# VITA-Group/MLSP

Measured on AMD Instinct MI355X. Metric: points/sec fwd+bwd, DGCNN+MLSP B=32 N=1024 k=20, higher is better.
Workload: dtype f32; 1 GPU; DGCNN encoder + 3 MLSP heads + losses, fwd+bwd+Adam, B=32/GPU N=1024 k=20 fp32 (BASELINE.json configs[1]), dropout 0.5, BN train; global_batch=32, points_per_cloud=1024, k=20, parallelism=dp1

## Files before the change

mlsp_amd/csrc/api.hip:

```cpp
#include "common.h"
#include "../../include/mlsp_hip.h"

#define CHECK(x) do { int _r = (x); if (_r != MLSP_OK) return _r; } while (0)
#define SLAB_BOUND_FLOATS ((size_t)16 << 20)

#include <mutex>
#include <unordered_map>
hipError_t mlsp_lds_limit(const void* fn, size_t lds) {
    static std::mutex mu;
    static std::unordered_map<uint64_t, size_t> raised;
    int dev = 0;
    (void)hipGetDevice(&dev);
    const uint64_t key = (uint64_t)(uintptr_t)fn * 64u + (uint64_t)(dev & 63);
    std::lock_guard<std::mutex> lk(mu);
    auto it = raised.find(key);
    if (it != raised.end() && it->second >= lds) return hipSuccess;
    const hipError_t e = hipFuncSetAttribute(fn, hipFuncAttributeMaxDynamicSharedMemorySize, (int)lds);
    if (e == hipSuccess) raised[key] = lds;
    return e;
}

extern "C" {

int mlsp_abi_version(void) { return MLSP_ABI_VERSION; }
// ... 157 lines not shown
    PREC_SCOPE(precision);
    if (!x || !idx || !W || !gamma || !beta || !out || !uv || !msel || !argsel || !s1 || !bn_save) return MLSP_ERR_ARG;
    if (B <= 0 || N <= 0 || C <= 0 || Cout <= 0 || k <= 0 || k > 255 || ldx < C || ldo < Cout) return MLSP_ERR_ARG;
    const int P = B * N;
    Workspace w(ws, ws_bytes);
    float* Wd = Wd_out ? Wd_out : w.take<float>((size_t)2 * Cout * C);
    int nparts = edge_reduce_parts(P);
    double* part = w.take<double>((size_t)nparts * 2 * Cout);
    GemmOpts so; take_slab(w, so, gemm_slab_floats(P, 2 * Cout, C));
    if (!w.ok()) return MLSP_ERR_WORKSPACE;
    float* scale = bn_save, *shift = bn_save + Cout, *mean = bn_save + 2 * Cout, *invstd = bn_save + 3 * Cout;
    if (!training) {
        if (!run_mean || !run_var) return MLSP_ERR_ARG;
        CHECK(launch_build_wd_eval(st, W, Cout, C, Wd, Cout, gamma, beta, run_mean, run_var, bn_save, 0, nullptr, nullptr, nullptr, nullptr, nullptr, eps));
    } else CHECK(launch_build_wd(st, W, Cout, C, Wd, (C >= 128 && C % 32 == 0 && build_wd_leaves_bound(Cout, C)) ? amax_reserve(Wd, 2 * Cout, C, C) : nullptr));
    CHECK(launch_gemm(st, false, true, P, 2 * Cout, C, x, ldx, Wd, C, uv, 2 * Cout, so));
    {
        const int tok = prof_cls_begin(st, MLSP_PROF_EDGE_REDUCE);
        const int rc = launch_edge_reduce(st, uv, idx, gamma, P, N, Cout, k, msel, argsel, s1, part, &nparts);
        prof_cls_end(st, tok, (double)P * (Cout * 4.0 + k * 4.0 + Cout * 9.0));
        if (rc != MLSP_OK) return rc;
    }
    if (training) {
        CHECK(launch_bn_finalize(st, part, nparts, (double)P * k, Cout, gamma, beta, run_mean, run_var, momentum, eps, scale,
                                 shift, mean, invstd, amax_offered_output(out, P, Cout, ldo, Cout)));
    }
    CHECK(launch_edge_select_act(st, msel, uv, P, Cout, scale, shift, act, slope, out, ldo));
    return MLSP_OK;
}

int mlsp_edgeconv_bwd_f32(const float* dOut, int lddo, const float* x, int ldx, const int32_t* rev_off, const int32_t* rev_ent,
                          const float* W, const float* out, int ldo, const float* uv, const float* msel, const uint8_t* argsel,
                          const float* s1, const float* bn_save, const float* Wd_in, int act, float slope, int training, int B, int N, int C,
                          int Cout, int k, float* dx, int lddx, int dx_accumulate, float* dW, float* dgamma, float* dbeta, int precision, void* ws,
                          size_t ws_bytes, mlsp_stream_t st) {
    PREC_SCOPE(precision);
    if (!dOut || !x || !rev_off || !rev_ent || !W || !out || !uv || !msel || !argsel || !s1 || !bn_save || !dW || !dgamma ||
        !dbeta)
        return MLSP_ERR_ARG;
    if (B <= 0 || N <= 0 || C <= 0 || Cout <= 0 || k <= 0 || ldx < C || lddo < Cout || ldo < Cout || (dx && lddx < C)) return MLSP_ERR_ARG;
    const int P = B * N;
    Workspace w(ws, ws_bytes);
    float* Wd = Wd_in ? nullptr : w.take<float>((size_t)2 * Cout * C);
    float* dWd = w.take<float>((size_t)2 * Cout * C);
    float* gz = w.take<float>((size_t)P * Cout);
    float* duv = w.take<float>((size_t)P * 2 * Cout);
    int nparts = bn_parts_max(P);
    double* part = w.take<double>((size_t)nparts * 2 * Cout);
    float* mean_dz = w.take<float>(Cout);
    float* mean_dzy = w.take<float>(Cout);
    GemmOpts so; take_slab(w, so, gemm_slab_floats(P, C, 2 * Cout), gemm_slab_floats(2 * Cout, C, P));
    if (!w.ok()) return MLSP_ERR_WORKSPACE;
    const float* scale = bn_save, *mean = bn_save + 2 * Cout, *invstd = bn_save + 3 * Cout;
    float* duv_amax = (C % 128 == 0 && edge_bwd_leaves_duv_bound(dOut, out, msel, uv, s1, argsel, Cout, scale, mean, invstd, gz, duv, lddo, ldo))
                          ? amax_reserve(duv, P, 2 * Cout, 2 * Cout) : nullptr;
    CHECK(launch_edge_bwd_reduce(st, dOut, out, msel, uv, P, Cout, mean, invstd, act, slope, part, lddo, ldo, duv_amax));
    CHECK(launch_bn_bwd_finalize(st, part, edge_bwd_reduce_parts(P, Cout, dOut, out, msel, uv, mean, invstd, lddo, ldo), (double)P * k, Cout,
                                 dgamma, dbeta, mean_dz, mean_dzy));
    const float* mdz = training ? mean_dz : nullptr;
    CHECK(launch_edge_bwd_point(st, dOut, out, uv, s1, P, Cout, k, scale, mean, invstd, mdz, mean_dzy, act, slope, gz, duv, lddo, ldo, duv_amax));
    CHECK(launch_edge_bwd_gather(st, gz, argsel, uv, rev_off, rev_ent, P, N, Cout, scale, mean, invstd, mdz, mean_dzy, duv, duv_amax));
    const float* Wdc = Wd_in;
    if (!Wdc && dx) { CHECK(launch_build_wd(st, W, Cout, C, Wd)); Wdc = Wd; }
    GemmOpts od = so; od.accumulate = dx_accumulate != 0;
    if (dx) CHECK(launch_gemm(st, false, false, P, C, 2 * Cout, duv, 2 * Cout, Wdc, C, dx, lddx, od));
    bool unfolded = false;
    GemmOpts ow = so; ow.unfold_dw = dW; ow.unfolded = &unfolded;
    CHECK(launch_gemm(st, true, false, 2 * Cout, C, P, duv, 2 * Cout, x, ldx, dWd, C, ow));
    if (!unfolded) CHECK(launch_unbuild_wd(st, dWd, Cout, C, dW));
    return MLSP_OK;
}

int mlsp_tnet_edge_fwd_f32(const float* x, int ldx, const int32_t* idx, const float* W1, const float* gamma1, const float* beta1,
                           float* run_mean1, float* run_var1, const float* W2, const float* gamma2, const float* beta2,
                           float* run_mean2, float* run_var2, float momentum, float eps, float slope, int training, int B, int N,
                           int C, int C1, int C2, int k, float* out, float* uv, float* s1, float* bn1_save, float* zsel,
                           uint8_t* argsel, float* bn2_save, int precision, void* ws, size_t ws_bytes, mlsp_stream_t st) {
    PREC_SCOPE(precision);
    if (!x || !idx || !W1 || !gamma1 || !beta1 || !W2 || !gamma2 || !beta2 || !out || !uv || !s1 || !bn1_save || !zsel || !argsel ||
        !bn2_save)
        return MLSP_ERR_ARG;
    if (B <= 0 || N <= 0 || C <= 0 || k <= 0 || ldx < C) return MLSP_ERR_ARG;
    if (C1 != 64 || C2 != 128 || tnet_points_per_tile(k) <= 0) return MLSP_ERR_UNSUPPORTED;
    const int P = B * N;
    Workspace w(ws, ws_bytes);
    float* Wd = w.take<float>((size_t)2 * C1 * C);
    float* msel = w.take<float>((size_t)P * C1);
    uint8_t* arg1 = w.take<uint8_t>((size_t)P * C1);
    int np1 = edge_reduce_parts(P), np2 = tnet_fwd_parts(B, N, k);
    double* part = w.take<double>((size_t)(np1 > np2 ? np1 : np2) * 2 * C2);
    GemmOpts so; take_slab(w, so, gemm_slab_floats(P, 2 * C1, C));
    if (!w.ok()) return MLSP_ERR_WORKSPACE;
    if (!training) {
        if (!run_mean1 || !run_var1 || !run_mean2 || !run_var2) return MLSP_ERR_ARG;
        CHECK(launch_build_wd_eval(st, W1, C1, C, Wd, C1, gamma1, beta1, run_mean1, run_var1, bn1_save, C2, gamma2, beta2, run_mean2, run_var2, bn2_save, eps));
    } else CHECK(launch_build_wd(st, W1, C1, C, Wd));
    CHECK(launch_gemm(st, false, true, P, 2 * C1, C, x, ldx, Wd, C, uv, 2 * C1, so));
    CHECK(launch_edge_reduce(st, uv, idx, gamma1, P, N, C1, k, msel, arg1, s1, part, &np1));
    if (training) {
        CHECK(launch_bn_finalize(st, part, np1, (double)P * k, C1, gamma1, beta1, run_mean1, run_var1, momentum, eps, bn1_save,
                                 bn1_save + C1, bn1_save + 2 * C1, bn1_save + 3 * C1));
    }
    {
        const int tok = prof_cls_begin(st, MLSP_PROF_TNET_FWD);
        const int rc = launch_tnet_edge_fwd(st, uv, idx, bn1_save, W2, gamma2, P, N, k, slope, zsel, argsel, part);
        prof_cls_end(st, tok, 2.0 * P * (double)k * C1 * C2);
        if (rc != MLSP_OK) return rc;
    }
    if (training) {
        CHECK(launch_bn_finalize(st, part, np2, (double)P * k, C2, gamma2, beta2, run_mean2, run_var2, momentum, eps, bn2_save,
                                 bn2_save + C2, bn2_save + 2 * C2, bn2_save + 3 * C2, amax_offered_output(out, P, C2, C2, C2)));
    }
    CHECK(launch_tnet_out(st, zsel, bn2_save, P, slope, out));
    return MLSP_OK;
// ... 782 lines not shown
```

mlsp_amd/csrc/edge.hip:

```cpp
#include "common.h"
#include <math.h>
#include <cstdlib>

#define EDGE_PTS_PER_WAVE 16

__global__ __launch_bounds__(256) void build_wd_kernel(const float* __restrict__ W, int Cout, int C, float* __restrict__ Wd, float* __restrict__ amax) {
    __shared__ float sm[4];
    int t = blockIdx.x * blockDim.x + threadIdx.x;
    float m = 0.f;
    if (t < Cout * C) {
        int o = t / C, c = t % C;
        float wa = W[(size_t)o * 2 * C + c], wb = W[(size_t)o * 2 * C + C + c];
        Wd[(size_t)o * C + c] = wa;
        Wd[(size_t)(Cout + o) * C + c] = wb - wa;
        m = fmaxf(fabsf(wa), fabsf(wb - wa));
    }
    if (!amax) return;
#pragma unroll
    for (int o = 1; o < 64; o <<= 1) m = fmaxf(m, __shfl_xor(m, o, 64));
    if ((threadIdx.x & 63) == 0) sm[threadIdx.x >> 6] = m;
    __syncthreads();
    if (threadIdx.x == 0) amax[blockIdx.x] = fmaxf(fmaxf(sm[0], sm[1]), fmaxf(sm[2], sm[3]));
    if (blockIdx.x == 0 && threadIdx.x >= gridDim.x) amax[threadIdx.x] = 0.f;
}
// ... 281 lines not shown
        for (int s0 = 0; s0 < KMAX; s0 += KC) {
            int jr[KC];
            if (EXACT && (KC % 4) == 0) {
#pragma unroll
                for (int s4 = 0; s4 < KC / 4; ++s4) {
                    const int4 t = *(const int4*)(irow + s0 + 4 * s4);
                    jr[4 * s4] = t.x; jr[4 * s4 + 1] = t.y; jr[4 * s4 + 2] = t.z; jr[4 * s4 + 3] = t.w;
                }
            } else {
#pragma unroll
                for (int s = 0; s < KC; ++s) jr[s] = (EXACT || s0 + s < k) ? irow[s0 + s] : 0;
            }
#pragma unroll
            for (int s = 0; s < KC; ++s) {
                if (EXACT || s0 + s < k) {
                    const f32x4 t = *(const f32x4*)(Us + jr[s] * CS + 4 * q);
                    const f32x2 ta = {t[0], t[1]}, tb = {t[2], t[3]};
                    s1a += ta; s1b += tb;
                    s2a = __builtin_elementwise_fma(ta, ta, s2a); s2b = __builtin_elementwise_fma(tb, tb, s2b);
#pragma unroll
                    for (int e = 0; e < 4; ++e) {
                        const bool take = (s0 + s == 0) || (t[e] > best[e]);
                        best[e] = take ? t[e] : best[e]; bs[e] = take ? s0 + s : bs[e];
                    }
                }
            }
        }
        const float s1[4] = {s1a[0] * sg[0], s1a[1] * sg[1], s1b[0] * sg[2], s1b[1] * sg[3]}, s2[4] = {s2a[0], s2a[1], s2b[0], s2b[1]};
        f32x4 b4, s4;
        uint32_t a4 = 0;
#pragma unroll
        for (int e = 0; e < 4; ++e) {
            b4[e] = best[e] * sg[e]; s4[e] = s1[e]; a4 |= (uint32_t)(bs[e] & 255) << (8 * e);
            ps[e] += (double)s1[e] + (double)k * v[e];
            pq[e] += (double)s2[e] + 2.0 * (double)v[e] * s1[e] + (double)k * v[e] * v[e];
        }
        *(f32x4*)(msel + i * Cout + c0 + 4 * q) = b4;
        *(f32x4*)(s1out + i * Cout + c0 + 4 * q) = s4;
        *(uint32_t*)(argsel + i * Cout + c0 + 4 * q) = a4;
    }
    __syncthreads();
    double* red = (double*)esm;
#pragma unroll
    for (int e = 0; e < 4; ++e) { red[(0 * PL + pl) * CS + 4 * q + e] = ps[e]; red[(1 * PL + pl) * CS + 4 * q + e] = pq[e]; }
    __syncthreads();
    if (tid < 2 * CS) {
        const int which = tid / CS, c = tid % CS;
        double a = 0.0;
        for (int u = 0; u < PL; ++u) a += red[(which * PL + u) * CS + c];
        part[((size_t)(b * psplit + ch) * 2 + which) * Cout + c0 + c] = a;
    }
}

__device__ __forceinline__ void edge_amax_raise(float* __restrict__ amax, float m) {
    __shared__ float wm[4];
#pragma unroll
    for (int o = 1; o < 64; o <<= 1) m = fmaxf(m, __shfl_xor(m, o, 64));
    if ((threadIdx.x & 63) == 0) wm[threadIdx.x >> 6] = m;
    __syncthreads();
    if (threadIdx.x == 0) atomicMax((unsigned int*)amax + (blockIdx.x & 255), __float_as_uint(fmaxf(fmaxf(wm[0], wm[1]), fmaxf(wm[2], wm[3]))));
}

template <int LR>
__global__ __launch_bounds__(256) void edge_bwd_gather_vec_kernel(const float* __restrict__ gz, const uint8_t* __restrict__ argsel,
                                                                  const float* __restrict__ uv, const int* __restrict__ rev_off,
                                                                  const int* __restrict__ rev_ent, int P, int N,
                                                                  const float* __restrict__ scale, const float* __restrict__ mean,
                                                                  const float* __restrict__ invstd,
                                                                  const float* __restrict__ mean_dz,
                                                                  const float* __restrict__ mean_dzy, float* __restrict__ duv,
                                                                  float* __restrict__ duv_amax) {
    constexpr int Cout = LR * 4, NP = 64 / LR;
    const int lane = threadIdx.x & 63;
    const int w = __builtin_amdgcn_readfirstlane(threadIdx.x >> 6);
    int j = blockIdx.x * 4 + w;
    if (N % 4 == 0) {
        int cloud, chunk;
        xcd_cloud_map(blockIdx.x, N / 4, P / N, cloud, chunk);
        j = cloud * N + chunk * 4 + w;
    }
    float pm = 0.f;
    if (j < P) {
        const int sub = lane / LR, c = (lane % LR) * 4;
        const int base = (j / N) * N;
        const int e0 = rev_off[j], e1 = rev_off[j + 1];
        const int ld = 2 * Cout;
        float A[4] = {0, 0, 0, 0}, Bc[4] = {0, 0, 0, 0};
        if (mean_dz) {
#pragma unroll
            for (int e = 0; e < 4; ++e) { float sc = scale[c + e]; A[e] = sc * mean_dz[c + e]; Bc[e] = sc * invstd[c + e] * mean_dzy[c + e]; }
        }
        float acc[4] = {0, 0, 0, 0};
        for (int ec = e0; ec < e1; ec += 64) {
            const int nent = min(64, e1 - ec);
            const int entv = lane < nent ? rev_ent[ec + lane] : 0;
            for (int t0 = 0; t0 < nent; t0 += NP) {
                const int t = t0 + sub;
                const bool ok = t < nent;
                const int ent = __shfl(entv, ok ? t : 0, 64);
                const int i = base + (ent >> 8), slot = ent & 255;
                const f32x4 g = *(const f32x4*)(gz + (size_t)i * Cout + c);
                const uint32_t a4 = *(const uint32_t*)(argsel + (size_t)i * Cout + c);
                const f32x4 v = *(const f32x4*)(uv + (size_t)i * ld + Cout + c);
#pragma unroll
                for (int e = 0; e < 4; ++e) {
                    float ge = (((a4 >> (8 * e)) & 255) == (uint32_t)slot) ? g[e] : 0.f;
                    acc[e] += ok ? (ge - Bc[e] * v[e]) : 0.f;
                }
            }
        }
#pragma unroll
        for (int o = LR; o < 64; o <<= 1)
#pragma unroll
// ... 117 lines not shown
    }
}

__global__ __launch_bounds__(256) void edge_select_act_vec_kernel(const float* __restrict__ msel, const float* __restrict__ uv,
                                                                  size_t total4, int C4, const float* __restrict__ scale,
                                                                  const float* __restrict__ shift, int act, float slope,
                                                                  float* __restrict__ out, int ldo) {
    for (size_t v = blockIdx.x * (size_t)blockDim.x + threadIdx.x; v < total4; v += (size_t)gridDim.x * blockDim.x) {
        const size_t i = v / C4; const int c = (int)(v % C4) * 4;
        const f32x4 m = *(const f32x4*)(msel + v * 4), vv = *(const f32x4*)(uv + i * 8 * C4 + 4 * C4 + c);
        const f32x4 sc = *(const f32x4*)(scale + c), sh = *(const f32x4*)(shift + c);
        f32x4 o;
#pragma unroll
        for (int e = 0; e < 4; ++e) o[e] = lrelu_or_relu(fmaf(m[e] + vv[e], sc[e], sh[e]), act, slope);
        *(f32x4*)(out + i * ldo + c) = o;
    }
}

__global__ __launch_bounds__(256) void edge_bwd_point_vec_kernel(const float* __restrict__ dOut, const float* __restrict__ out,
                                                                 const float* __restrict__ uv, const float* __restrict__ s1,
                                                                 size_t total4, int C4, int k, const float* __restrict__ scale,
                                                                 const float* __restrict__ mean, const float* __restrict__ invstd,
                                                                 const float* __restrict__ mean_dz, const float* __restrict__ mean_dzy,
                                                                 int act, float slope, float* __restrict__ gz,
                                                                 float* __restrict__ duv, int lddo, int ldo,
                                                                 float* __restrict__ duv_amax) {
    const float fk = (float)k;
    float pm = 0.f;
    for (size_t v = blockIdx.x * (size_t)blockDim.x + threadIdx.x; v < total4; v += (size_t)gridDim.x * blockDim.x) {
        const size_t i = v / C4; const int c = (int)(v % C4) * 4;
        const f32x4 d4 = *(const f32x4*)(dOut + i * lddo + c), o4 = *(const f32x4*)(out + i * ldo + c);
        const f32x4 sc = *(const f32x4*)(scale + c);
        f32x4 g, dv;
#pragma unroll
        for (int e = 0; e < 4; ++e) {
            float d = d4[e];
            if (act && !(o4[e] > 0.f)) d *= (act == 1 ? 0.f : slope);
            g[e] = sc[e] * d; dv[e] = g[e];
        }
        if (mean_dz) {
            const f32x4 vv = *(const f32x4*)(uv + i * 8 * C4 + 4 * C4 + c), s4 = *(const f32x4*)(s1 + v * 4);
#pragma unroll
            for (int e = 0; e < 4; ++e) {
                float A = sc[e] * mean_dz[c + e], Bc = sc[e] * invstd[c + e] * mean_dzy[c + e];
                dv[e] = g[e] - fk * A - Bc * (s4[e] + fk * (vv[e] - mean[c + e]));
            }
        }
        *(f32x4*)(gz + v * 4) = g;
        *(f32x4*)(duv + i * 8 * C4 + 4 * C4 + c) = dv;
#pragma unroll
        for (int e = 0; e < 4; ++e) pm = fmaxf(pm, fabsf(dv[e]));
    }
    if (duv_amax) edge_amax_raise(duv_amax, pm);
}

__global__ __launch_bounds__(256) void edge_bwd_gather_kernel(const float* __restrict__ gz, const uint8_t* __restrict__ argsel,
                                                              const float* __restrict__ uv, const int* __restrict__ rev_off,
                                                              const int* __restrict__ rev_ent, int P, int N, int Cout,
                                                              const float* __restrict__ scale, const float* __restrict__ mean,
                                                              const float* __restrict__ invstd,
                                                              const float* __restrict__ mean_dz,
                                                              const float* __restrict__ mean_dzy, float* __restrict__ duv) {
    const int lane = threadIdx.x & 63;
    const int w = __builtin_amdgcn_readfirstlane(threadIdx.x >> 6);
    const int j = blockIdx.x * 4 + w;
    if (j >= P) return;
    const int base = (j / N) * N;
    const int e0 = rev_off[j], e1 = rev_off[j + 1];
    const int ld = 2 * Cout;
    for (int c = lane; c < Cout; c += 64) {
        float A = 0.f, Bc = 0.f;
        if (mean_dz) { float sc = scale[c]; A = sc * mean_dz[c]; Bc = sc * invstd[c] * mean_dzy[c]; }
        float acc = 0.f;
        for (int e = e0; e < e1; ++e) {
            int ent = rev_ent[e];
            int i = base + (ent >> 8), slot = ent & 255;
            size_t t = (size_t)i * Cout + c;
            float g = (argsel[t] == slot) ? gz[t] : 0.f;
            acc += g - Bc * uv[(size_t)i * ld + Cout + c];
        }
        float u = uv[(size_t)j * ld + c];
        duv[(size_t)j * ld + c] = acc - (float)(e1 - e0) * (A + Bc * (u - mean[c]));
    }
}

__global__ __launch_bounds__(256) void graph_feature_fwd_kernel(const float* __restrict__ x, const int* __restrict__ idx,
                                                                int P, int N, int C, int k, float* __restrict__ F) {
    size_t total = (size_t)P * k * C;
    for (size_t t = blockIdx.x * (size_t)blockDim.x + threadIdx.x; t < total; t += (size_t)gridDim.x * blockDim.x) {
        int c = (int)(t % C);
        size_t e = t / C;
        size_t i = e / k;
        int j = (int)(i / N) * N + idx[e];
        float xi = x[i * C + c];
        F[e * 2 * C + c] = x[(size_t)j * C + c] - xi;
        F[e * 2 * C + C + c] = xi;
    }
}

__global__ __launch_bounds__(256) void graph_feature_bwd_kernel(const float* __restrict__ dF, const int* __restrict__ rev_off,
                                                                const int* __restrict__ rev_ent, int P, int N, int C, int k,
                                                                float* __restrict__ dx) {
    size_t total = (size_t)P * C;
    for (size_t t = blockIdx.x * (size_t)blockDim.x + threadIdx.x; t < total; t += (size_t)gridDim.x * blockDim.x) {
        int c = (int)(t % C);
        size_t i = t / C;
// ... 72 lines not shown
        int psplit = 1;
        while (psplit < 8 && (B * nsl * psplit < 512 || (N / psplit) * k * 2 > 16 * 1024) && N % (psplit * 2) == 0) psplit *= 2;
        const size_t lds = (size_t)N * ELDS_CS * sizeof(float) + align_up((size_t)((N + psplit - 1) / psplit) * k * 2, 16);
        if (lds <= 150 * 1024 && B * psplit <= edge_reduce_parts(P) && lds >= (size_t)2 * (256 / (ELDS_CS / 4)) * ELDS_CS * sizeof(double)) {
            auto kern = k == 20 ? edge_reduce_lds_kernel<20, true> : k <= 20 ? edge_reduce_lds_kernel<20, false> : k <= 32 ? edge_reduce_lds_kernel<32, false>
                      : k == 40 ? edge_reduce_lds_kernel<40, true> : edge_reduce_lds_kernel<40, false>;
            if (lds > 64 * 1024) {
                hipError_t e = mlsp_lds_limit((const void*)kern, lds);
                if (e != hipSuccess) return (int)e;
            }
            hipLaunchKernelGGL(kern, dim3(B * nsl * psplit), dim3(256), lds, st, uv, idx, gamma, B, N, k, Cout, psplit, msel, argsel, s1, part);
            if (nparts_used) *nparts_used = B * psplit;
            return mlsp_launch_status();
        }
    }
    if (al && (Cout == 64 || Cout == 128 || Cout == 256)) {
        dim3 g(edge_reduce_parts(P)), b(256);
        if (Cout == 64) hipLaunchKernelGGL((edge_reduce_vec_kernel<16>), g, b, 0, st, uv, idx, gamma, P, N, k, msel, argsel, s1, part);
        else if (Cout == 128) hipLaunchKernelGGL((edge_reduce_vec_kernel<32>), g, b, 0, st, uv, idx, gamma, P, N, k, msel, argsel, s1, part);
        else hipLaunchKernelGGL((edge_reduce_vec_kernel<64>), g, b, 0, st, uv, idx, gamma, P, N, k, msel, argsel, s1, part);
        return mlsp_launch_status();
    }
    size_t lds = (size_t)8 * Cout * sizeof(double);
    if (lds > 64 * 1024) return MLSP_ERR_UNSUPPORTED;
    hipLaunchKernelGGL(edge_reduce_kernel, dim3(edge_reduce_parts(P)), dim3(256), lds, st, uv, idx, gamma, P, N, Cout, k,
                       msel, argsel, s1, part);
    return mlsp_launch_status();
}
int launch_edge_select_act(hipStream_t st, const float* msel, const float* uv, int P, int Cout, const float* scale,
                           const float* shift, int act, float slope, float* out, int ldo) {
    if (Cout % 4 == 0 && ldo % 4 == 0 && ((((uintptr_t)msel | (uintptr_t)uv | (uintptr_t)out | (uintptr_t)scale | (uintptr_t)shift) & 15) == 0)) {
        size_t t4 = (size_t)P * Cout / 4;
        hipLaunchKernelGGL(edge_select_act_vec_kernel, dim3(ew_blocks2(t4)), dim3(256), 0, st, msel, uv, t4, Cout / 4, scale, shift,
                           act, slope, out, ldo);
        return mlsp_launch_status();
    }
    hipLaunchKernelGGL(edge_select_act_kernel, dim3(ew_blocks2((size_t)P * Cout)), dim3(256), 0, st, msel, uv, P, Cout, scale,
                       shift, act, slope, out, ldo);
    return mlsp_launch_status();
}
static bool edge_bwd_reduce_vec_ok(const float* dOut, const float* out, const float* msel, const float* uv, int Cout, const float* mean,
                                   const float* invstd, int lddo, int ldo) {
    return Cout % 4 == 0 && Cout <= 1024 && 256 % (Cout / 4) == 0 && lddo % 4 == 0 && ldo % 4 == 0 &&
           ((((uintptr_t)dOut | (uintptr_t)out | (uintptr_t)msel | (uintptr_t)uv | (uintptr_t)mean | (uintptr_t)invstd) & 15) == 0);
}
static bool edge_bwd_point_vec_ok(const float* dOut, const float* out, const float* uv, const float* s1, int Cout, const float* scale,
                                  const float* gz, const float* duv, int lddo, int ldo) {
    return Cout % 4 == 0 && lddo % 4 == 0 && ldo % 4 == 0 &&
           ((((uintptr_t)dOut | (uintptr_t)out | (uintptr_t)uv | (uintptr_t)s1 | (uintptr_t)gz | (uintptr_t)duv | (uintptr_t)scale) & 15) == 0);
}
static bool edge_bwd_gather_vec_ok(const float* gz, const uint8_t* argsel, const float* uv, int Cout, const float* duv) {
    return (((uintptr_t)uv | (uintptr_t)gz | (uintptr_t)duv) & 15) == 0 && (((uintptr_t)argsel) & 3) == 0 && (Cout == 64 || Cout == 128 || Cout == 256);
}
bool edge_bwd_leaves_duv_bound(const float* dOut, const float* out, const float* msel, const float* uv, const float* s1, const uint8_t* argsel,
                               int Cout, const float* scale, const float* mean, const float* invstd, const float* gz, const float* duv,
                               int lddo, int ldo) {
    return edge_bwd_reduce_vec_ok(dOut, out, msel, uv, Cout, mean, invstd, lddo, ldo) &&
           edge_bwd_point_vec_ok(dOut, out, uv, s1, Cout, scale, gz, duv, lddo, ldo) && edge_bwd_gather_vec_ok(gz, argsel, uv, Cout, duv);
}
int launch_edge_bwd_reduce(hipStream_t st, const float* dOut, const float* out, const float* msel, const float* uv, int P,
                           int Cout, const float* mean, const float* invstd, int act, float slope, double* part, int lddo, int ldo,
                           float* duv_amax) {
    if (edge_bwd_reduce_vec_ok(dOut, out, msel, uv, Cout, mean, invstd, lddo, ldo)) {
        hipLaunchKernelGGL(edge_bwd_reduce_vec_kernel, dim3((P + EVROWS - 1) / EVROWS), dim3(256), 0, st, dOut, out, msel, uv, P, Cout,
                           mean, invstd, act, slope, part, lddo, ldo, duv_amax);
        return mlsp_launch_status();
    }
    hipLaunchKernelGGL(edge_bwd_reduce_kernel, dim3((Cout + 63) / 64, (P + 511) / 512), dim3(256), 0, st, dOut, out, msel, uv,
                       P, Cout, mean, invstd, act, slope, part, lddo, ldo);
    return mlsp_launch_status();
}
int launch_edge_bwd_point(hipStream_t st, const float* dOut, const float* out, const float* uv, const float* s1, int P,
                          int Cout, int k, const float* scale, const float* mean, const float* invstd, const float* mean_dz,
                          const float* mean_dzy, int act, float slope, float* gz, float* duv, int lddo, int ldo, float* duv_amax) {
    if (edge_bwd_point_vec_ok(dOut, out, uv, s1, Cout, scale, gz, duv, lddo, ldo)) {
        size_t t4 = (size_t)P * Cout / 4;
        hipLaunchKernelGGL(edge_bwd_point_vec_kernel, dim3(ew_blocks2(t4)), dim3(256), 0, st, dOut, out, uv, s1, t4, Cout / 4, k, scale,
                           mean, invstd, mean_dz, mean_dzy, act, slope, gz, duv, lddo, ldo, duv_amax);
        return mlsp_launch_status();
    }
    hipLaunchKernelGGL(edge_bwd_point_kernel, dim3(ew_blocks2((size_t)P * Cout)), dim3(256), 0, st, dOut, out, uv, s1, P, Cout,
                       k, scale, mean, invstd, mean_dz, mean_dzy, act, slope, gz, duv, lddo, ldo);
    return mlsp_launch_status();
}
int launch_edge_bwd_gather(hipStream_t st, const float* gz, const uint8_t* argsel, const float* uv, const int* rev_off,
                           const int* rev_ent, int P, int N, int Cout, const float* scale, const float* mean,
                           const float* invstd, const float* mean_dz, const float* mean_dzy, float* duv, float* duv_amax) {
    if (edge_bwd_gather_vec_ok(gz, argsel, uv, Cout, duv)) {
        dim3 g((P + 3) / 4), b(256);
        if (Cout == 64) hipLaunchKernelGGL((edge_bwd_gather_vec_kernel<16>), g, b, 0, st, gz, argsel, uv, rev_off, rev_ent, P, N, scale, mean, invstd, mean_dz, mean_dzy, duv, duv_amax);
        else if (Cout == 128) hipLaunchKernelGGL((edge_bwd_gather_vec_kernel<32>), g, b, 0, st, gz, argsel, uv, rev_off, rev_ent, P, N, scale, mean, invstd, mean_dz, mean_dzy, duv, duv_amax);
        else hipLaunchKernelGGL((edge_bwd_gather_vec_kernel<64>), g, b, 0, st, gz, argsel, uv, rev_off, rev_ent, P, N, scale, mean, invstd, mean_dz, mean_dzy, duv, duv_amax);
        return mlsp_launch_status();
    }
    hipLaunchKernelGGL(edge_bwd_gather_kernel, dim3((P + 3) / 4), dim3(256), 0, st, gz, argsel, uv, rev_off, rev_ent, P, N,
                       Cout, scale, mean, invstd, mean_dz, mean_dzy, duv);
    return mlsp_launch_status();
}
int launch_graph_feature_fwd(hipStream_t st, const float* x, const int* idx, int P, int N, int C, int k, float* F) {
    hipLaunchKernelGGL(graph_feature_fwd_kernel, dim3(ew_blocks2((size_t)P * k * C)), dim3(256), 0, st, x, idx, P, N, C, k, F);
    return mlsp_launch_status();
}
int launch_graph_feature_bwd(hipStream_t st, const float* dF, const int* rev_off, const int* rev_ent, int P, int N, int C,
                             int k, float* dx) {
    hipLaunchKernelGGL(graph_feature_bwd_kernel, dim3(ew_blocks2((size_t)P * C)), dim3(256), 0, st, dF, rev_off, rev_ent, P, N,
                       C, k, dx);
    return mlsp_launch_status();
}
```

mlsp_amd/csrc/launchers.h:

```cpp
#pragma once

hipError_t mlsp_lds_limit(const void* fn, size_t lds);

int gemm_precision_mode();
float* amax_reserve(const float* X, long rows, int cols, int ld);
float* amax_offered_output(const float* out, long rows, int cols, int ld, int need);
int launch_slab_reduce(hipStream_t st, const float* slab, float* C, int M, int N, int ldc, int nsplit, float* unfold_dw = nullptr,
                       bool* unfolded = nullptr);
int gemm_stat_parts(int M, int N, int K);
int gemm_panel_rows(int M, int N, int K);
size_t gemm_slab_floats(int M, int N, int K);
int prof_cls_begin(hipStream_t st, int cls);
void prof_cls_end(hipStream_t st, int token, double work);
bool gemm_xf_supported(bool ta, bool tb, int M, int N, int K, const float* A, int lda, const float* B, int ldb, int which);
int gemm_bs_parts(int M, int N, int K, int lda, int ldb, int ldc);
bool gemm_dy_supported(bool ta, bool tb, int M, int N, int K, const float* A, int lda, const float* B, int ldb);
bool gemm_xf_on_split(bool ta, bool tb, int M, int N, int K, int which);
int launch_gemm(hipStream_t st, bool ta, bool tb, int M, int N, int K, const float* A, int lda, const float* B, int ldb, float* C, int ldc,
                const GemmOpts& o = GemmOpts());
int launch_gemm_mx(hipStream_t st, bool ta, bool tb, int M, int N, int K, const void* A, int a_bf16, int lda, const void* B, int b_bf16, int ldb,
                   void* C, int c_bf16, int ldc, const GemmOpts& o = GemmOpts());

int launch_knn(hipStream_t st, const float* x, int ld, int B, int N, int C, int k, int* idx, float* xx_ws, void* planes, size_t plane_bytes);
int launch_group_reverse(hipStream_t st, const int* idx, int B, int S, int N, int k, int* rev_off, int* rev_ent);
// ... 21 lines not shown
                              float* run_mean, float* run_var, float momentum, float eps, float* scale, float* shift, float* save_mean,
                              float* save_invstd, float* gsum, int ppg);
int launch_bn_eval_prepare(hipStream_t st, int C, const float* gamma, const float* beta, const float* run_mean, const float* run_var, float eps,
                           float* scale, float* shift, float* save_mean, float* save_invstd);
int launch_bn_act_fwd(hipStream_t st, const float* Y, float* Z, size_t rows, int C, const float* scale, const float* shift, int act, float slope,
                      float p_drop, uint64_t seed);
int launch_bn_act_bwd(hipStream_t st, const float* dZ, const float* Y, float* dY, int M, int C, const float* scale, const float* shift,
                      const float* mean, const float* invstd, int training, int act, float slope, float p_drop, uint64_t seed, double* part,
                      float* dgamma, float* dbeta, float* mean_dz, float* mean_dzy, float* zero_vec, float* gpart = nullptr,
                      int rows_per_group = 0, int* gpart_slabs = nullptr, const double* pre_stats = nullptr, int pre_parts = 0);
int launch_bn_bwd_finalize_coef_z(hipStream_t st, const double* part, int nparts, double count, int C, const float* bn_save, float* dgamma,
                                  float* dbeta, float* coef, float* zero_vec);
int launch_bn_bwd_finalize_coef_groups(hipStream_t st, const double* part, int nparts, double count, int C, const float* bn_save, float* dgamma,
                                       float* dbeta, float* coef, const float* gys, int ppg, int rows, float* gout);
int launch_bn_bwd_finalize_z(hipStream_t st, const double* part, int nparts, double count, int C, float* dgamma, float* dbeta, float* mean_dz,
                             float* mean_dzy, float* zero_vec);
int launch_bn_bwd_finalize(hipStream_t st, const double* part, int nparts, double count, int C, float* dgamma, float* dbeta, float* mean_dz,
                           float* mean_dzy);
int launch_colsum_groups(hipStream_t st, const float* X, int G, int rows_per_group, int C, float* out, float* scratch = nullptr);
int launch_bn_dy_gbias(hipStream_t st, const float* Y, int G, int rows_per_group, int C, const double* stats, int panel_rows, const float* coef,
                       float* scratch, float* out, const float* ysum);
int launch_colsum_groups_fin(hipStream_t st, const float* scratch, int G, int C, int slabs, float* out);
int launch_colsum(hipStream_t st, const float* X, int M, int C, double* part, float* out);
int launch_bn_act_bwd_partials_vec(hipStream_t st, const float* dZ, const float* Y, int M, int C, const float* scale, const float* shift,
                                   const float* mean, const float* invstd, int act, float slope, double* part);
int launch_colmax_fwd(hipStream_t st, const float* Z, int B, int N, int C, float* out, int* arg);
int launch_colmax_bwd(hipStream_t st, const float* dOut, const int* arg, int B, int N, int C, float* dZ);
int launch_segmax_fwd(hipStream_t st, const float* Z, int P, int k, int C, float* out, uint8_t* argk);
int launch_segsel_act_fwd(hipStream_t st, const float* Y, int G, int k, int C, const float* scale, const float* shift, int act, float slope,
                          float* out, float* ysel, uint8_t* argk);
int launch_segsel_bwd_apply(hipStream_t st, const float* dOut, const float* Y, const float* ysel, const uint8_t* argk, size_t M, int k, int C,
                            const float* bn, const float* m1, const float* m2, int act, float slope, float* dY);
int launch_segmax_bwd(hipStream_t st, const float* dOut, const uint8_t* argk, int P, int k, int C, float* dZ);
int launch_bn_act_fwd_b16(hipStream_t st, const void* Y, void* Z, int rows, int C, const float* scale, const float* shift, int act, float slope,
                          float p_drop, uint64_t seed);
int launch_bn_act_bwd_b16(hipStream_t st, const void* dZ, const void* Y, void* dY, int M, int C, const float* scale, const float* shift,
                          const float* mean, const float* invstd, int training, int act, float slope, float p_drop, uint64_t seed, double* part,
                          float* dgamma, float* dbeta, float* mean_dz, float* mean_dzy, float* zero_vec);
int launch_colsum_groups_b16(hipStream_t st, const void* X, int G, int rows_per_group, int C, float* out, float* scratch);

int edge_bwd_reduce_parts(int P, int Cout, const void* a, const void* b, const void* c, const void* d, const void* e, const void* f, int lddo,
                          int ldo);
int edge_reduce_parts(int P);
bool build_wd_leaves_bound(int Cout, int C);
int launch_build_wd(hipStream_t st, const float* W, int Cout, int C, float* Wd, float* amax = nullptr);
int launch_build_wd_eval(hipStream_t st, const float* W, int Cout, int C, float* Wd, int Ca, const float* ga, const float* ba, const float* rma,
                         const float* rva, float* sva, int Cb, const float* gb, const float* bb, const float* rmb, const float* rvb, float* svb,
                         float eps);
int launch_unbuild_wd(hipStream_t st, const float* dWd, int Cout, int C, float* dW);
int launch_edge_reduce(hipStream_t st, const float* uv, const int* idx, const float* gamma, int P, int N, int Cout, int k, float* msel,
                       uint8_t* argsel, float* s1, double* part, int* nparts_used);
int launch_edge_select_act(hipStream_t st, const float* msel, const float* uv, int P, int Cout, const float* scale, const float* shift, int act,
                           float slope, float* out, int ldo);
bool edge_bwd_leaves_duv_bound(const float* dOut, const float* out, const float* msel, const float* uv, const float* s1, const uint8_t* argsel,
                               int Cout, const float* scale, const float* mean, const float* invstd, const float* gz, const float* duv, int lddo,
                               int ldo);
int launch_edge_bwd_reduce(hipStream_t st, const float* dOut, const float* out, const float* msel, const float* uv, int P, int Cout,
                           const float* mean, const float* invstd, int act, float slope, double* part, int lddo, int ldo, float* duv_amax);
int launch_edge_bwd_point(hipStream_t st, const float* dOut, const float* out, const float* uv, const float* s1, int P, int Cout, int k,
                          const float* scale, const float* mean, const float* invstd, const float* mean_dz, const float* mean_dzy, int act,
                          float slope, float* gz, float* duv, int lddo, int ldo, float* duv_amax);
int launch_edge_bwd_gather(hipStream_t st, const float* gz, const uint8_t* argsel, const float* uv, const int* rev_off, const int* rev_ent, int P,
                           int N, int Cout, const float* scale, const float* mean, const float* invstd, const float* mean_dz, const float* mean_dzy,
                           float* duv, float* duv_amax);
int launch_graph_feature_fwd(hipStream_t st, const float* x, const int* idx, int P, int N, int C, int k, float* F);
int launch_graph_feature_bwd(hipStream_t st, const float* dF, const int* rev_off, const int* rev_ent, int P, int N, int C, int k, float* dx);

int launch_chamfer_fwd(hipStream_t st, const float* pred, const float* gold, const float* mask, int B, int N, float scale, float* per_cloud,
                       int* argA, int* argB, float* loss);
int launch_chamfer_bwd(hipStream_t st, const float* pred, const float* gold, const float* mask, int B, int N, float scale, const float* per_cloud,
                       const int* argA, const int* argB, const float* gout, float* dpred);
int launch_chamfer_dir_fwd(hipStream_t st, const float* p1, const float* p2, const float* mc, int B, int N, float* per_cloud, int* arg, float* loss);
int launch_chamfer_dir_bwd(hipStream_t st, const float* p1, const float* p2, const float* mc, int B, int N, const float* per_cloud, const int* arg,
                           const float* gout, float* dp1, float* dp2);
int launch_normal_loss_fwd(hipStream_t st, const float* pred, const float* gt, const float* w, int P, float weight, double* part, float* out);
int launch_normal_loss_bwd(hipStream_t st, const float* pred, const float* gt, const float* w, int P, float weight, const float* fwd_out,
                           const float* gout, float* dpred);
int launch_density_tail_fwd(hipStream_t st, const float* logits, const float* w, int P, int nc, float* pvec, float* dens);
int launch_density_tail_bwd(hipStream_t st, const float* pvec, const float* w, const float* dp, const float* dd, int P, int nc, float* dlogits);
int launch_density_loss_fwd(hipStream_t st, const float* pvec, const float* dens, const float* tvec, const float* target, const float* m, int P,
                            int nc, float dweight, double* part, float* out);
int launch_density_loss_bwd(hipStream_t st, const float* pvec, const float* dens, const float* tvec, const float* target, const float* m, int P,
                            int nc, float dweight, const float* fwd_out, const float* gkl, const float* gmae, float* dp, float* dd);

int tnet_grid(int ntiles);
int tnet_points_per_tile(int k);
int tnet_fwd_parts(int B, int N, int k);
int launch_tnet_edge_fwd(hipStream_t st, const float* uv, const int* idx, const float* bn1, const float* W2, const float* gamma2, int P, int N, int k,
                         float slope, float* zsel, uint8_t* argsel, double* part);
int launch_tnet_out(hipStream_t st, const float* zsel, const float* bn2, int P, float slope, float* out);
int launch_tnet_bwd_reduce(hipStream_t st, const float* dT, const float* T, const float* zsel, const float* bn2, int P, float slope, double* part);
int launch_tnet_bwd_g(hipStream_t st, const float* dT, const float* T, const float* bn2, const float* mean_dz, const float* mean_dzy, int P,
                      float slope, float* g, float* coef);
size_t tnet_bwd_scratch_floats(int ntiles);
int launch_tnet_edge_bwd(hipStream_t st, const float* uv, const int* idx, const float* bn1, const float* W2, const float* bn2, const float* g,
                         const uint8_t* argsel, const float* coef, int P, int N, int k, float slope, float* dhp, float* scratch, double* part1,
                         float* dW2, int* nparts);
int launch_tnet_edge_bwd2(hipStream_t st, const float* dhp, const float* uv, const float* s1, const float* bn1, const float* m1, const float* m2,
                          const int* rev_off, const int* rev_ent, int P, int N, int k, float* duv);
size_t tnet_w1_moment_doubles(int P, int k);
int launch_tnet_bwd_w1_moments(hipStream_t st, const float* dhp, const int* idx, const int* rev_off, const float* x, int ldx, const float* W1,
                               const float* bn1, const float* m1, const float* m2, int P, int N, int k, int C, double* scratch, float* dW1);

int launch_colsel(hipStream_t st, const float* Y, const float* gamma, int B, int N, int C, float* ysel, int* arg);
int launch_colsel_panels(hipStream_t st, const float* pv, const int* pr, const float* gamma, int B, int N, int C, int panel_rows, float* ysel,
                         int* arg, const float* bn, int act, float slope, float* out);
int launch_colsel_out(hipStream_t st, const float* ysel, const float* bn, int B, int C, int act, float slope, float* out);
int launch_colmax_bwd_coef(hipStream_t st, const float* dOut, const float* out, const float* ysel, const float* bn, int B, int C, double count,
                           int act, float slope, int training, float* g, float* coef, float* dgamma, float* dbeta);
// ... 120 lines not shown
```

Measured before the change: 8.528 million points/s.

## Fuse edge-conv backward point and gather into one LDS-resident wide kernel

Adds a fused edge-conv backward kernel. Each block loads a whole cloud's gradient, argsel and v-features for a 16-channel slice into LDS (up to about 150KB), then computes both the point-wise dv term and the reverse-neighbor gather du term from LDS. This drops the intermediate gz buffer round-trip through global memory and one kernel launch. Points with many reverse neighbors (more than 64) are handled by a second wave-cooperative pass. The trade-off is heavy LDS use with 1024-thread blocks, which limits occupancy, and each block redundantly stages the full cloud when the points are split across blocks.

```diff
diff --git a/mlsp_amd/csrc/api.hip b/mlsp_amd/csrc/api.hip
--- a/mlsp_amd/csrc/api.hip
+++ b/mlsp_amd/csrc/api.hip
@@ -233,14 +233,19 @@
     GemmOpts so; take_slab(w, so, gemm_slab_floats(P, C, 2 * Cout), gemm_slab_floats(2 * Cout, C, P));
     if (!w.ok()) return MLSP_ERR_WORKSPACE;
     const float* scale = bn_save, *mean = bn_save + 2 * Cout, *invstd = bn_save + 3 * Cout;
-    float* duv_amax = (C % 128 == 0 && edge_bwd_leaves_duv_bound(dOut, out, msel, uv, s1, argsel, Cout, scale, mean, invstd, gz, duv, lddo, ldo))
+    float* duv_amax = (C % 128 == 0 && edge_bwd_leaves_duv_bound(dOut, out, msel, uv, s1, argsel, P, N, Cout, scale, mean, invstd, gz, duv, lddo, ldo))
                           ? amax_reserve(duv, P, 2 * Cout, 2 * Cout) : nullptr;
     CHECK(launch_edge_bwd_reduce(st, dOut, out, msel, uv, P, Cout, mean, invstd, act, slope, part, lddo, ldo, duv_amax));
     CHECK(launch_bn_bwd_finalize(st, part, edge_bwd_reduce_parts(P, Cout, dOut, out, msel, uv, mean, invstd, lddo, ldo), (double)P * k, Cout,
                                  dgamma, dbeta, mean_dz, mean_dzy));
     const float* mdz = training ? mean_dz : nullptr;
-    CHECK(launch_edge_bwd_point(st, dOut, out, uv, s1, P, Cout, k, scale, mean, invstd, mdz, mean_dzy, act, slope, gz, duv, lddo, ldo, duv_amax));
-    CHECK(launch_edge_bwd_gather(st, gz, argsel, uv, rev_off, rev_ent, P, N, Cout, scale, mean, invstd, mdz, mean_dzy, duv, duv_amax));
+    if (edge_bwd_wide_ok(dOut, out, uv, s1, argsel, scale, duv, P, N, Cout, lddo, ldo)) {
+        CHECK(launch_edge_bwd_wide(st, dOut, out, uv, s1, argsel, rev_off, rev_ent, P, N, Cout, k, scale, mean, invstd, mdz, mean_dzy, act, slope,
+                                   duv, lddo, ldo, duv_amax));
+    } else {
+        CHECK(launch_edge_bwd_point(st, dOut, out, uv, s1, P, Cout, k, scale, mean, invstd, mdz, mean_dzy, act, slope, gz, duv, lddo, ldo, duv_amax));
+        CHECK(launch_edge_bwd_gather(st, gz, argsel, uv, rev_off, rev_ent, P, N, Cout, scale, mean, invstd, mdz, mean_dzy, duv, duv_amax));
+    }
     const float* Wdc = Wd_in;
     if (!Wdc && dx) { CHECK(launch_build_wd(st, W, Cout, C, Wd)); Wdc = Wd; }
     GemmOpts od = so; od.accumulate = dx_accumulate != 0;
diff --git a/mlsp_amd/csrc/edge.hip b/mlsp_amd/csrc/edge.hip
--- a/mlsp_amd/csrc/edge.hip
+++ b/mlsp_amd/csrc/edge.hip
@@ -357,13 +357,19 @@
     }
 }
 
+template <int NW = 4>
 __device__ __forceinline__ void edge_amax_raise(float* __restrict__ amax, float m) {
-    __shared__ float wm[4];
+    __shared__ float wm[NW];
 #pragma unroll
     for (int o = 1; o < 64; o <<= 1) m = fmaxf(m, __shfl_xor(m, o, 64));
     if ((threadIdx.x & 63) == 0) wm[threadIdx.x >> 6] = m;
     __syncthreads();
-    if (threadIdx.x == 0) atomicMax((unsigned int*)amax + (blockIdx.x & 255), __float_as_uint(fmaxf(fmaxf(wm[0], wm[1]), fmaxf(wm[2], wm[3]))));
+    if (threadIdx.x == 0) {
+        float t = wm[0];
+#pragma unroll
+        for (int u = 1; u < NW; ++u) t = fmaxf(t, wm[u]);
+        atomicMax((unsigned int*)amax + (blockIdx.x & 255), __float_as_uint(t));
+    }
 }
 
 template <int LR>
@@ -587,6 +593,164 @@
         for (int e = 0; e < 4; ++e) pm = fmaxf(pm, fabsf(dv[e]));
     }
     if (duv_amax) edge_amax_raise(duv_amax, pm);
+}
+
+#define EBW_LONG 64
+#define EBW_BATCH 8
+#define EBW_LDS_MAX ((size_t)150 * 1024)
+template <int CS, int NT, bool TRAIN>
+__global__ __launch_bounds__(NT) void edge_bwd_wide_kernel(const float* __restrict__ dOut, const float* __restrict__ out,
+                                                           const float* __restrict__ uv, const float* __restrict__ s1,
+                                                           const uint8_t* __restrict__ argsel, const int* __restrict__ rev_off,
+                                                           const int* __restrict__ rev_ent, int B, int N, int Cout, int k, int psplit,
+                                                           const float* __restrict__ scale, const float* __restrict__ mean,
+                                                           const float* __restrict__ invstd, const float* __restrict__ mean_dz,
+                                                           const float* __restrict__ mean_dzy, int act, float slope,
+                                                           float* __restrict__ duv, int lddo, int ldo, float* __restrict__ duv_amax) {
+    extern __shared__ __attribute__((aligned(16))) float esm[];
+    constexpr int QPP = CS / 4, PL = NT / QPP, NS = 64 / QPP;
+    float* Gs = esm;
+    uint32_t* As = (uint32_t*)(esm + (size_t)N * CS);
+    float* Vs = (float*)(As + (size_t)N * QPP);
+    const int tid = threadIdx.x;
+    const int nsl = Cout / CS, bpc = nsl * psplit;
+    int b, r;
+    xcd_cloud_map(blockIdx.x, bpc, B, b, r);
+    const int sl = r % nsl, ch = r / nsl;
+    const int c0 = sl * CS, ld = 2 * Cout;
+    const int pper = (N + psplit - 1) / psplit, pbeg = ch * pper, pend = min(N, pbeg + pper);
+    const int q = tid % QPP, pl = tid / QPP, c = c0 + 4 * q;
+    const size_t p0 = (size_t)b * N;
+    const f32x4 sc = *(const f32x4*)(scale + c);
+    for (int row = pl; row < N; row += 4 * PL) {
+        f32x4 d4[4], o4[4], v4[4];
+        uint32_t a4[4];
+#pragma unroll
+        for (int u = 0; u < 4; ++u) {
+            const size_t i = p0 + row + u * PL;
+            if (row + u * PL < N) {
+                d4[u] = *(const f32x4*)(dOut + i * lddo + c); o4[u] = *(const f32x4*)(out + i * ldo + c);
+                a4[u] = *(const uint32_t*)(argsel + i * Cout + c);
+                if (TRAIN) v4[u] = *(const f32x4*)(uv + i * ld + Cout + c);
+            }
+        }
+#pragma unroll
+        for (int u = 0; u < 4; ++u) {
+            const int rw = row + u * PL;
+            if (rw < N) {
+                f32x4 g;
+#pragma unroll
+                for (int e = 0; e < 4; ++e) {
+                    float d = d4[u][e];
+                    if (act && !(o4[u][e] > 0.f)) d *= (act == 1 ? 0.f : slope);
+                    g[e] = sc[e] * d;
+                }
+                *(f32x4*)(Gs + rw * CS + 4 * q) = g;
+                As[rw * QPP + q] = a4[u];
+                if (TRAIN) *(f32x4*)(Vs + rw * CS + 4 * q) = v4[u];
+            }
+        }
+    }
+    __syncthreads();
+    const float fk = (float)k;
+    float A[4] = {0, 0, 0, 0}, Bc[4] = {0, 0, 0, 0}, mu[4] = {0, 0, 0, 0};
+    if (TRAIN) {
+#pragma unroll
+        for (int e = 0; e < 4; ++e) { A[e] = sc[e] * mean_dz[c + e]; Bc[e] = sc[e] * invstd[c + e] * mean_dzy[c + e]; mu[e] = mean[c + e]; }
+    }
+    float pm = 0.f;
+    for (int il = pbeg + pl; il < pend; il += PL) {
+        const size_t j = p0 + il;
+        const int e0 = rev_off[j], e1 = rev_off[j + 1];
+        const f32x4 g = *(const f32x4*)(Gs + il * CS + 4 * q);
+        f32x4 dv = g;
+        if (TRAIN) {
+            const f32x4 vv = *(const f32x4*)(Vs + il * CS + 4 * q), s4 = *(const f32x4*)(s1 + j * Cout + c);
+#pragma unroll
+            for (int e = 0; e < 4; ++e) dv[e] = g[e] - fk * A[e] - Bc[e] * (s4[e] + fk * (vv[e] - mu[e]));
+        }
+        *(f32x4*)(duv + j * ld + Cout + c) = dv;
+#pragma unroll
+        for (int e = 0; e < 4; ++e) pm = fmaxf(pm, fabsf(dv[e]));
+        if (e1 - e0 > EBW_LONG) continue;
+        float acc[4] = {0, 0, 0, 0};
+        for (int eb = e0; eb < e1; eb += EBW_BATCH) {
+            int ent[EBW_BATCH];
+#pragma unroll
+            for (int u = 0; u < EBW_BATCH; ++u) ent[u] = eb + u < e1 ? rev_ent[eb + u] : -1;
+#pragma unroll
+            for (int u = 0; u < EBW_BATCH; ++u) {
+                const bool ok = ent[u] >= 0;
+                const int i = ok ? ent[u] >> 8 : 0;
+                const uint32_t slot = (uint32_t)ent[u] & 255u;
+                const f32x4 gi = *(const f32x4*)(Gs + i * CS + 4 * q);
+                const uint32_t a4 = As[i * QPP + q];
+                f32x4 vi = {0.f, 0.f, 0.f, 0.f};
+                if (TRAIN) vi = *(const f32x4*)(Vs + i * CS + 4 * q);
+#pragma unroll
+                for (int e = 0; e < 4; ++e) {
+                    const float ge = (((a4 >> (8 * e)) & 255u) == slot) ? gi[e] : 0.f;
+                    acc[e] += ok ? (TRAIN ? ge - Bc[e] * vi[e] : ge) : 0.f;
+                }
+            }
+        }
+        f32x4 o4;
+        if (TRAIN) {
+            const f32x4 u = *(const f32x4*)(uv + j * ld + c);
+#pragma unroll
+            for (int e = 0; e < 4; ++e) o4[e] = acc[e] - (float)(e1 - e0) * (A[e] + Bc[e] * (u[e] - mu[e]));
+        } else {
+#pragma unroll
+            for (int e = 0; e < 4; ++e) o4[e] = acc[e];
+        }
+        *(f32x4*)(duv + j * ld + c) = o4;
+#pragma unroll
+        for (int e = 0; e < 4; ++e) pm = fmaxf(pm, fabsf(o4[e]));
+    }
+    {
+        const int sub = (tid & 63) / QPP;
+        const int w = __builtin_amdgcn_readfirstlane(tid >> 6);
+        for (int il = pbeg + w; il < pend; il += NT / 64) {
+            const size_t j = p0 + il;
+            const int e0 = rev_off[j], e1 = rev_off[j + 1];
+            if (e1 - e0 <= EBW_LONG) continue;
+            float acc[4] = {0, 0, 0, 0};
+            for (int eb = e0; eb < e1; eb += NS) {
+                const bool ok = eb + sub < e1;
+                const int ent = ok ? rev_ent[eb + sub] : 0;
+                const int i = ent >> 8;
+                const uint32_t slot = (uint32_t)ent & 255u;
+                const f32x4 gi = *(const f32x4*)(Gs + i * CS + 4 * q);
+                const uint32_t a4 = As[i * QPP + q];
+                f32x4 vi = {0.f, 0.f, 0.f, 0.f};
+                if (TRAIN) vi = *(const f32x4*)(Vs + i * CS + 4 * q);
+#pragma unroll
+                for (int e = 0; e < 4; ++e) {
+                    const float ge = (((a4 >> (8 * e)) & 255u) == slot) ? gi[e] : 0.f;
+                    acc[e] += ok ? (TRAIN ? ge - Bc[e] * vi[e] : ge) : 0.f;
+                }
+            }
+#pragma unroll
+            for (int o = QPP; o < 64; o <<= 1)
+#pragma unroll
+                for (int e = 0; e < 4; ++e) acc[e] += __shfl_xor(acc[e], o, 64);
+            if (sub == 0) {
+                f32x4 o4;
+                if (TRAIN) {
+                    const f32x4 u = *(const f32x4*)(uv + j * ld + c);
+#pragma unroll
+                    for (int e = 0; e < 4; ++e) o4[e] = acc[e] - (float)(e1 - e0) * (A[e] + Bc[e] * (u[e] - mu[e]));
+                } else {
+#pragma unroll
+                    for (int e = 0; e < 4; ++e) o4[e] = acc[e];
+                }
+                *(f32x4*)(duv + j * ld + c) = o4;
+#pragma unroll
+                for (int e = 0; e < 4; ++e) pm = fmaxf(pm, fabsf(o4[e]));
+            }
+        }
+    }
+    if (duv_amax) edge_amax_raise<NT / 64>(duv_amax, pm);
 }
 
 __global__ __launch_bounds__(256) void edge_bwd_gather_kernel(const float* __restrict__ gz, const uint8_t* __restrict__ argsel,
@@ -765,11 +929,39 @@
 static bool edge_bwd_gather_vec_ok(const float* gz, const uint8_t* argsel, const float* uv, int Cout, const float* duv) {
     return (((uintptr_t)uv | (uintptr_t)gz | (uintptr_t)duv) & 15) == 0 && (((uintptr_t)argsel) & 3) == 0 && (Cout == 64 || Cout == 128 || Cout == 256);
 }
+#define EBW_CS 16
+static bool edge_bwd_wide_fits(int N, int Cout) { return Cout % EBW_CS == 0 && (size_t)N * EBW_CS * 9 <= EBW_LDS_MAX; }
+bool edge_bwd_wide_ok(const float* dOut, const float* out, const float* uv, const float* s1, const uint8_t* argsel, const float* scale,
+                      const float* duv, int P, int N, int Cout, int lddo, int ldo) {
+    return N > 0 && P % N == 0 && N % 4 == 0 && Cout % 4 == 0 && lddo % 4 == 0 && ldo % 4 == 0 && edge_bwd_wide_fits(N, Cout) &&
+           ((((uintptr_t)dOut | (uintptr_t)out | (uintptr_t)uv | (uintptr_t)s1 | (uintptr_t)duv | (uintptr_t)scale) & 15) == 0) &&
+           (((uintptr_t)argsel) & 3) == 0;
+}
 bool edge_bwd_leaves_duv_bound(const float* dOut, const float* out, const float* msel, const float* uv, const float* s1, const uint8_t* argsel,
-                               int Cout, const float* scale, const float* mean, const float* invstd, const float* gz, const float* duv,
-                               int lddo, int ldo) {
+                               int P, int N, int Cout, const float* scale, const float* mean, const float* invstd, const float* gz,
+                               const float* duv, int lddo, int ldo) {
     return edge_bwd_reduce_vec_ok(dOut, out, msel, uv, Cout, mean, invstd, lddo, ldo) &&
-           edge_bwd_point_vec_ok(dOut, out, uv, s1, Cout, scale, gz, duv, lddo, ldo) && edge_bwd_gather_vec_ok(gz, argsel, uv, Cout, duv);
+           (edge_bwd_wide_ok(dOut, out, uv, s1, argsel, scale, duv, P, N, Cout, lddo, ldo) ||
+            (edge_bwd_point_vec_ok(dOut, out, uv, s1, Cout, scale, gz, duv, lddo, ldo) && edge_bwd_gather_vec_ok(gz, argsel, uv, Cout, duv)));
+}
+int launch_edge_bwd_wide(hipStream_t st, const float* dOut, const float* out, const float* uv, const float* s1, const uint8_t* argsel,
+                         const int* rev_off, const int* rev_ent, int P, int N, int Cout, int k, const float* scale, const float* mean,
+                         const float* invstd, const float* mean_dz, const float* mean_dzy, int act, float slope, float* duv, int lddo,
+                         int ldo, float* duv_amax) {
+    if (!edge_bwd_wide_ok(dOut, out, uv, s1, argsel, scale, duv, P, N, Cout, lddo, ldo)) return MLSP_ERR_UNSUPPORTED;
+    constexpr int NT = 1024, CS = EBW_CS;
+    const int B = P / N, nsl = Cout / CS;
+    int psplit = 1;
+    while (psplit < 8 && B * nsl * psplit < 256) psplit *= 2;
+    const bool train = mean_dz != nullptr;
+    const size_t lds = (size_t)N * CS * (train ? 9 : 5);
+#define EBW_GO(TR) do { auto kern = edge_bwd_wide_kernel<CS, NT, TR>; \
+        if (lds > 64 * 1024) { hipError_t e_ = mlsp_lds_limit((const void*)kern, lds); if (e_ != hipSuccess) return (int)e_; } \
+        hipLaunchKernelGGL(kern, dim3(B * nsl * psplit), dim3(NT), lds, st, dOut, out, uv, s1, argsel, rev_off, rev_ent, B, N, Cout, k, psplit, \
+                           scale, mean, invstd, mean_dz, mean_dzy, act, slope, duv, lddo, ldo, duv_amax); } while (0)
+    if (train) EBW_GO(true); else EBW_GO(false);
+#undef EBW_GO
+    return mlsp_launch_status();
 }
 int launch_edge_bwd_reduce(hipStream_t st, const float* dOut, const float* out, const float* msel, const float* uv, int P,
                            int Cout, const float* mean, const float* invstd, int act, float slope, double* part, int lddo, int ldo,
diff --git a/mlsp_amd/csrc/launchers.h b/mlsp_amd/csrc/launchers.h
--- a/mlsp_amd/csrc/launchers.h
+++ b/mlsp_amd/csrc/launchers.h
@@ -97,9 +97,15 @@
                        uint8_t* argsel, float* s1, double* part, int* nparts_used);
 int launch_edge_select_act(hipStream_t st, const float* msel, const float* uv, int P, int Cout, const float* scale, const float* shift, int act,
                            float slope, float* out, int ldo);
+bool edge_bwd_wide_ok(const float* dOut, const float* out, const float* uv, const float* s1, const uint8_t* argsel, const float* scale,
+                      const float* duv, int P, int N, int Cout, int lddo, int ldo);
 bool edge_bwd_leaves_duv_bound(const float* dOut, const float* out, const float* msel, const float* uv, const float* s1, const uint8_t* argsel,
-                               int Cout, const float* scale, const float* mean, const float* invstd, const float* gz, const float* duv, int lddo,
-                               int ldo);
+                               int P, int N, int Cout, const float* scale, const float* mean, const float* invstd, const float* gz,
+                               const float* duv, int lddo, int ldo);
+int launch_edge_bwd_wide(hipStream_t st, const float* dOut, const float* out, const float* uv, const float* s1, const uint8_t* argsel,
+                         const int* rev_off, const int* rev_ent, int P, int N, int Cout, int k, const float* scale, const float* mean,
+                         const float* invstd, const float* mean_dz, const float* mean_dzy, int act, float slope, float* duv, int lddo,
+                         int ldo, float* duv_amax);
 int launch_edge_bwd_reduce(hipStream_t st, const float* dOut, const float* out, const float* msel, const float* uv, int P, int Cout,
                            const float* mean, const float* invstd, int act, float slope, double* part, int lddo, int ldo, float* duv_amax);
 int launch_edge_bwd_point(hipStream_t st, const float* dOut, const float* out, const float* uv, const float* s1, int P, int Cout, int k,
```

Measured after the change: 8.593 million points/s (median of 6 runs). Within noise of the previous version (+0.8%).
